# wolearyc/ramannoodle

Measured on AMD Instinct MI355X. Metric: structures/sec (GNN polarizability eval), higher is better.
Workload: dtype f32

## Files before the change

### ramannoodle_amd/csrc/api.hip

```cpp
#include <hip/hip_runtime.h>

#include <algorithm>
#include <chrono>
#include <cmath>
#include <cstdarg>
#include <cstdio>
#include <cstdlib>
#include <cstring>
#include <functional>
#include <memory>
#include <mutex>
#include <string>
#include <thread>
#include <vector>

#include "../../include/rn_potgnn.h"
#include "graph_plan.hpp"
#include "kernels.hpp"
#include "weight_layout.hpp"

using namespace rn;

namespace {

// ... 8 lines not shown
  do {                                                 \
    hipError_t _e = (expr);                            \
    if (_e != hipSuccess) throw HipError{_e, #expr};   \
  } while (0)

struct DeviceBuf {
  void *p = nullptr;
  size_t bytes = 0;
  ~DeviceBuf() { release(); }
  void release() {
    if (p) (void)hipFree(p);
    p = nullptr;
    bytes = 0;
  }
  void ensure(size_t n) {
    if (n <= bytes) return;
    release();
    HIP_TRY(hipMalloc(&p, n));
    bytes = n;
  }
  template <typename T>
  T *as() const { return reinterpret_cast<T *>(p); }
};

enum KernelId {
  K_GEOM = 0, K_NODE_INIT, K_PROJ_NODE, K_PROJ_EDGE_C1, K_NODE_AGG, K_PROJ_EDGE_C3, K_PROJ_C2,
  K_EDGE_AGG, K_READOUT_MLP, K_READOUT_REDUCE, K_C2_PAIRS, K_COUNT
};
const char *kKernelNames[K_COUNT] = {
    "geom_rbf", "node_init", "proj_node", "proj_edge_c1", "node_agg", "proj_edge_c3",
    "proj_c2", "edge_agg", "readout_mlp", "readout_reduce", "c2_pairs"};

template <typename T>
struct Lane {
  hipStream_t stream = nullptr;
  hipEvent_t done = nullptr;
  DeviceBuf unit4, node[2], edge[2], npc1, np3, bufA, bufB;
  DeviceBuf fbA, fbB;
};

template <typename T>
struct Precision {
  bool ready = false;
  DeviceBuf weights;
  DeviceBuf lattice;
  std::vector<PassW<T>> pass;
  ReadoutW<T> ro{};
  const T *offsets = nullptr, *node_table = nullptr, *ones = nullptr;
  Lane<T> lanes[2];
  std::vector<DeviceBuf> snap_node, snap_edge;
  std::vector<DeviceBuf> tape_node, tape_edge, tape_agg;
  DeviceBuf bw[18];
  hipStream_t side = nullptr;
  hipEvent_t ev_side[3] = {nullptr, nullptr, nullptr};
  DeviceBuf tn_arena;
  DeviceBuf tape_z1, bn_stats, grad, seeds, mv, type_sums;
  DeviceBuf in_dcart, in_lat, in_grads;
  DeviceBuf eye_seeds;
  int eye_frames = 0;
  bool tape_on = false;
};

struct TimedLaunch {
  int kid;
  hipEvent_t a, b;
};

}

struct rn_potgnn {
  mutable std::recursive_mutex lock;
  rn_potgnn_config cfg{};
  Dims d{};
  int chunk = 1;
  size_t f64_budget = 0;
  bool keep_stages = false;
  bool snap_pairs = false;
  bool last_pair_rows = false;
  bool debug_sync = false;
  GraphPlan plan;
  bool split_projections = true;
  bool want_pair_rows = true;
  bool want_c2_pairs = true;
  DeviceBuf step_seg, step_stage;
  float *step_host = nullptr;
  bool tape_ps = true;
  bool mfma_f16 = true;
  bool mfma_f16_requested = true;
  bool mfma_range_fallback = false;
  Graph g{};
  DeviceBuf g_ints;
  DeviceBuf ps_fail;
  double lattice[9], mean[9], stdv[9];
  DeviceBuf d_mean_std;
  std::vector<float> packed;
  PackedLayout lay;
  Precision<float> f32;
  Precision<double> f64;
  DeviceBuf io_pos, io_alpha, io_vec6, io_lat, io_types;
  struct Slot {
    DeviceBuf pos, alpha;
    hipEvent_t copied = nullptr, done = nullptr;
    bool busy = false;
  } slots[2];
  hipStream_t copy_stream = nullptr, exec_stream = nullptr;
  int next_slot = 0;
  struct HostStage {
    float *pin[2] = {nullptr, nullptr};
    size_t elems = 0;
    hipEvent_t copied[2] = {nullptr, nullptr};
    hipEvent_t done = nullptr;
    DeviceBuf pos;
    DeviceBuf lat;
    hipEvent_t caller = nullptr;
    char *out_pin = nullptr;
    size_t out_bytes = 0;
  } hstage;
  int last_chunk_structs = 0;
  int train_S = 0;
  int train_prec = 4;
  bool train_lat = false, train_types = false;
  bool tape_fused = true;
  bool device_training = false;
  bool grads_on_device = false;
  bool host_stale = false;
  DeviceBuf adam_m, adam_v, trainable_mask, derived_ops;
  int num_derived_ops = 0, derived_first_stage = 0;
  double bn_count = 0;
  rn_potgnn_reduce_fn reducer = nullptr;
  void *reducer_ctx = nullptr;
  bool last_was_f64 = false;
  bool last_in_order = false;
  int profiling = 0;
  std::vector<TimedLaunch> timed;
  double k_ms[K_COUNT] = {0};
  int64_t k_launches[K_COUNT] = {0};
  std::string error;
  hipEvent_t ev_start = nullptr;
  hipEvent_t ev_g[2] = {nullptr, nullptr};
  bool interleave = true;
  std::vector<int32_t> grp_labels;
  int grp_G = 0;
  DeviceBuf grp_csr, grp_jac, grp_disp, grp_out;
  DeviceBuf mode_vectors;
  DeviceBuf grp_jl, grp_lat, cells_lat;
};

namespace {

void set_error(rn_potgnn *h, const char *fmt, ...) {
  char buf[512];
  va_list ap;
  va_start(ap, fmt);
  vsnprintf(buf, sizeof(buf), fmt, ap);
  va_end(ap);
  if (h) {
    std::lock_guard<std::recursive_mutex> hold(h->lock);
    h->error = buf;
  } else {
    g_create_error = buf;
  }
}

bool lean_workspace(const rn_potgnn *h);
size_t per_structure_elems(const rn_potgnn *h, bool lean);
template <typename T>
// ... 266 lines not shown
    }
    cur = 0;
    snapshot(0);
  }

  void run_stages() {
    begin();
    for (int p = 0; p < h->cfg.num_message_passes; ++p) {
      stage_project(p);
      stage_aggregate(p);
    }
  }

  void project(const T *X, int64_t R, int K, const T *WT, int NOUT, T *Y, const T *bias, int amode, const T *nd) {
    if constexpr (sizeof(T) == 4) {
      if (h->mfma_f16 && h->split_projections &&
          launch_rowgemm_split(X, K, K, R, WT, NOUT, Y, false, bias, amode, nd, h->g, st()))
        return;
    }
    launch_rowgemm<T>(X, R, K, WT, NOUT, Y, nullptr, bias, false, amode, nd, h->g, st());
  }

  void stage_project(int p) {
    const PassW<T> &w = prec<T>(h).pass[p];
    const Graph &g = h->g;
    const Dims d = h->d;
    const int nxt = cur ^ 1;
    target_tape(p + 1, nxt);
    if constexpr (sizeof(T) == 4) {
      if (narrow()) {
        Timer t(h, st(), K_NODE_AGG);
        launch_node_narrow(edge[cur], node[cur], node[nxt], S, g, d, w, st());
        return;
      }
    }
    {
      Timer t(h, st(), K_PROJ_NODE);
      if (node_centred()) project(node[cur], MN, d.FnP, w.c1_WnT_c, 2 * d.FnP, npc1, w.c1_bias_c, 0, nullptr);
      else project(node[cur], MN, d.FnP, w.c1_WnT, 2 * d.FnP, npc1, w.c1_bias, 0, nullptr);
    }
    bool node_fused = false;
    if constexpr (sizeof(T) == 4) {
      if (fused() && h->plan.use_node_fused) {
        Timer t(h, st(), K_NODE_AGG);
        if (node_centred() && g.na_num > 0) launch_node_atom(edge[cur], node[cur], npc1, node[nxt], S, g, d, w, st(), pair_rows());
        else launch_node_fused(edge[cur], node[cur], npc1, node[nxt], S, g, d, w, h->mfma_f16, node_centred(), st());
        node_fused = true;
      }
    }
    if (!node_fused) {
      {
        Timer t(h, st(), K_PROJ_EDGE_C1);
        project(edge[cur], ME, d.FeP, w.c1_WeT, 2 * d.FnP, bufA, nullptr, 0, nullptr);
      }
      {
        Timer t(h, st(), K_NODE_AGG);
        launch_node_agg<T>(npc1, bufA, node[cur], node[nxt], S, g, d, w, st());
      }
    }
    {
      Timer t(h, st(), K_PROJ_NODE);
      if (role_split(w)) project(node[nxt], MN, d.FnP, w.c3_WnT_c, 6 * d.FeP, np3, w.c3_nshift_c, 0, nullptr);
      else project(node[nxt], MN, d.FnP, w.c3_WnT, 6 * d.FeP, np3, w.c3_nshift, 0, nullptr);
    }
    if (!fused()) {
      {
        Timer t(h, st(), K_PROJ_EDGE_C3);
        project(edge[cur], ME, d.FeP, w.c3_WeT, 4 * d.FeP, bufB, nullptr, 0, nullptr);
      }
      {
        Timer t(h, st(), K_PROJ_C2);
        project(nullptr, ME, d.FnP, w.c2_WT, 2 * d.FeP, bufA, w.c2_bias, 1, node[nxt]);
      }
    }
  }

  void stage_aggregate(int p) {
    const PassW<T> &w = prec<T>(h).pass[p];
    const int nxt = cur ^ 1;
    const float *c2_rows = nullptr;
    if constexpr (sizeof(T) == 4) {
      if (c2_pairs(w)) {
        Timer t(h, st(), K_C2_PAIRS);
        launch_c2_pairs(node[nxt], bufA, S, h->g, h->d, w, st());
        c2_rows = bufA;
      }
    }
    {
      Timer t(h, st(), K_EDGE_AGG);
      if constexpr (sizeof(T) == 4) {
        if (narrow()) launch_edge_narrow(edge[cur], edge[nxt], node[nxt], S, h->g, h->d, w, st());
        else if (role_split(w)) launch_edge_ps(edge[cur], edge[nxt], node[nxt], np3, tape_agg(p), S, h->g, h->d, w, h->ps_fail.as<int>(), st(), pair_rows(), h->mfma_f16, c2_rows);
        else if (fused()) edge_unfused_in_blocks(p);
        else HIP_TRY(launch_edge_agg<T>(bufB, np3, bufA, edge[cur], edge[nxt], S, h->g, h->d, w, tape_agg(p), st()));
      } else {
        HIP_TRY(launch_edge_agg<T>(bufB, np3, bufA, edge[cur], edge[nxt], S, h->g, h->d, w, tape_agg(p), st()));
      }
    }
    cur = nxt;
    snapshot(p + 1);
  }

  void edge_unfused_in_blocks(int p) {
    const PassW<T> &w = prec<T>(h).pass[p];
    const Graph &g = h->g;
    const Dims d = h->d;
    const int nxt = cur ^ 1;
    const size_t per_frame = (size_t)g.E * (size_t)(6 * d.FeP) * sizeof(T);
    int block = (int)std::max<size_t>(1, std::min<size_t>((size_t)S, ((size_t)1 << 30) / std::max<size_t>(per_frame, 1)));
    if (const char *e = getenv("RN_POTGNN_UNFUSED_BLOCK_FRAMES")) block = std::max(1, std::min(block, atoi(e)));
    ln->fbA.ensure((size_t)block * g.E * 2 * d.FeP * sizeof(T));
    ln->fbB.ensure((size_t)block * g.E * 4 * d.FeP * sizeof(T));
    T *fa = ln->fbA.template as<T>(), *fb = ln->fbB.template as<T>();
    T *agg = tape_agg(p);
    for (int s0 = 0; s0 < S; s0 += block) {
      const int sb = std::min(block, S - s0);
      const int64_t rows = (int64_t)sb * g.E;
      const T *e_in = edge[cur] + (size_t)s0 * g.E * d.FeP, *nd = node[nxt] + (size_t)s0 * g.N * d.FnP;
      project(e_in, rows, d.FeP, w.c3_WeT, 4 * d.FeP, fb, nullptr, 0, nullptr);
      project(nullptr, rows, d.FnP, w.c2_WT, 2 * d.FeP, fa, w.c2_bias, 1, nd);
      HIP_TRY(launch_edge_agg<T>(fb, np3 + (size_t)s0 * g.N * 6 * d.FeP, fa, e_in, edge[nxt] + (size_t)s0 * g.E * d.FeP, sb, g, d, w,
                                 agg ? agg + (size_t)s0 * g.E * d.FeP : nullptr, st()));
    }
  }

  void finish() {
    Precision<T> &P = prec<T>(h);
    const Graph &g = h->g;
    const Dims d = h->d;
    if constexpr (sizeof(T) == 4) {
      if (narrow()) {
        Timer t(h, st(), K_READOUT_MLP);
        const double *ms = h->d_mean_std.as<double>();
        launch_readout_narrow(edge[cur], unit4, S, g, d, P.ro, ms, ms + 9, io.vec6, io.alpha, io.alpha_raw,
                              h->keep_stages ? bufA : nullptr, st());
        HIP_TRY(hipGetLastError());
        return;
      }
    }
    int pol_stride = 32;
    {
      Timer t(h, st(), K_READOUT_MLP);
      const int HP = std::max(d.FeP, 32);
      bool done = false;
      if constexpr (sizeof(T) == 4) {
        if (fused() && h->plan.use_readout_fused) {
          pol_stride = h->keep_stages ? 32 : 16;
          launch_readout_fused(edge[cur], ME, P.ro, bufA, h->mfma_f16, st(), pair_rows(), pol_stride);
          done = true;
        }
      }
      if (!done) {
        launch_rowgemm<T>(edge[cur], ME, d.FeP, P.ro.W0T, HP, bufA, P.ro.scale0, P.ro.shift0, true, 0,
                          nullptr, g, st());
        launch_rowgemm<T>(bufA, ME, HP, P.ro.W3T, HP, bufB, P.ones, P.ro.b3, true, 0, nullptr, g, st());
        launch_rowgemm<T>(bufB, ME, HP, P.ro.W5T, 32, bufA, nullptr, P.ro.b5, false, 0, nullptr, g,
                          st());
      }
    }
    {
      Timer t(h, st(), K_READOUT_REDUCE);
      const double *ms = h->d_mean_std.as<double>();
      launch_readout_reduce<T>(bufA, unit4, S, g, ms, ms + 9, io.vec6, io.alpha, io.alpha_raw, st(), pol_stride);
    }
    HIP_TRY(hipGetLastError());
  }
  bool fused() const { return sizeof(T) == 4 && h->plan.use_fused && (!prec<T>(h).tape_on || h->tape_fused); }
// ... 946 lines not shown
               o_nt = push(plan.nt.begin), o_bt = push(plan.bt.begin), o_pt = push(plan.pt.begin), o_ipos = push(plan.in_pos),
               o_pe = push(plan.pair_of_edge), o_pa = push(plan.pair_a), o_pb = push(plan.pair_b);
  buf.ensure(ints.size() * sizeof(int));
  HIP_TRY(hipMemcpy(buf.p, ints.data(), ints.size() * sizeof(int), hipMemcpyHostToDevice));
  const int *base = buf.as<int>();
  Graph g = plan.scalars();
  g.edge_a = base + o_a;
  g.edge_b = base + o_b;
  g.out_ptr = base + o_op;
  g.in_ptr = base + o_ip;
  g.in_edge = base + o_ie;
  g.in_pos = base + o_ipos;
  g.atom_type = base + o_at;
  g.rev_edge = base + o_rv;
  g.pair_of_edge = base + o_pe;
  g.pair_a = base + o_pa;
  g.pair_b = base + o_pb;
  g.tile_begin = base + o_tb;
  g.trip_off = base + o_to;
  g.nt_begin = base + o_nt;
  g.pt_begin = base + o_pt;
  g.bt_begin = base + o_bt;
  return g;
}

static void size_chunk(rn_potgnn *h) {
  int chunk = h->cfg.max_chunk_structures;
  if (const char *e = getenv("RN_POTGNN_CHUNK")) chunk = atoi(e);
  if (chunk <= 0) {
    const size_t per = per_structure_elems(h, lean_workspace(h)) * sizeof(float);
    size_t budget = (h->plan.use_fused || h->plan.use_narrow) ? ((size_t)8192 << 20) : ((size_t)1536 << 20);
    size_t free_b = 0, total_b = 0;
    if (hipMemGetInfo(&free_b, &total_b) == hipSuccess && free_b > 0)
      budget = std::min(budget, std::max<size_t>(free_b / 8 / (size_t)h->plan.num_lanes, (size_t)64 << 20));
    chunk = (int)std::max<size_t>(1, budget / std::max<size_t>(per, 1));
    chunk = std::min(chunk, 4096);
    h->f64_budget = (size_t)24 << 30;
    if (free_b > 0) h->f64_budget = std::min(h->f64_budget, std::max<size_t>(free_b / 8 / (size_t)h->plan.num_lanes, (size_t)64 << 20));
  }
  h->chunk = chunk;
}

int rn_potgnn_create(const rn_potgnn_config *cfg, const int32_t *edge_a, const int32_t *edge_b,
                     const int32_t *atom_types, const double *lattice, const float *weights,
                     size_t num_weights, const double *mean, const double *stddev,
                     rn_potgnn **out) {
  if (!out) return RN_ERR_INVALID_ARGUMENT;
  *out = nullptr;
  std::string invalid;
  int rc = validate_create_args(cfg, edge_a, edge_b, atom_types, !lattice || !weights || !mean || !stddev, &num_weights, invalid);
  if (rc != RN_OK) {
    set_error(nullptr, "%s", invalid.c_str());
    return rc;
  }

  int ndev = 0;
  if (hipGetDeviceCount(&ndev) != hipSuccess || ndev <= 0 || cfg->device < 0 ||
      cfg->device >= ndev) {
    set_error(nullptr, "no usable HIP device (count=%d, requested=%d)", ndev, cfg->device);
    return RN_ERR_NO_DEVICE;
  }
  int cus = 256;
  {
    hipDeviceProp_t prop;
    if (hipGetDeviceProperties(&prop, cfg->device) == hipSuccess && prop.multiProcessorCount > 0) cus = prop.multiProcessorCount;
  }

  std::unique_ptr<rn_potgnn> h(new rn_potgnn());
  h->cfg = *cfg;
  std::memcpy(h->lattice, lattice, sizeof(h->lattice));
  std::memcpy(h->mean, mean, sizeof(h->mean));
  std::memcpy(h->stdv, stddev, sizeof(h->stdv));
  h->snap_pairs = getenv("RN_POTGNN_KEEP_STAGES") && atoi(getenv("RN_POTGNN_KEEP_STAGES")) == 2;
  h->keep_stages = getenv("RN_POTGNN_KEEP_STAGES") && atoi(getenv("RN_POTGNN_KEEP_STAGES")) != 0 && !h->snap_pairs;
  h->debug_sync = getenv("RN_POTGNN_DEBUG_SYNC") && atoi(getenv("RN_POTGNN_DEBUG_SYNC")) != 0;
  if (const char *e = getenv("RN_POTGNN_INTERLEAVE")) h->interleave = atoi(e) != 0;
  if (const char *e = getenv("RN_POTGNN_MFMA")) h->mfma_f16_requested = !(e[0] == 'f' && e[1] == '3');
  h->mfma_f16 = h->mfma_f16_requested;
  if (const char *e = getenv("RN_POTGNN_TAPE_FUSED")) h->tape_fused = atoi(e) != 0;
  if (const char *e = getenv("RN_POTGNN_TAPE_PS")) h->tape_ps = atoi(e) != 0;
  h->split_projections = getenv("RN_POTGNN_SPLIT_PROJ") ? atoi(getenv("RN_POTGNN_SPLIT_PROJ")) != 0 : true;
  h->want_pair_rows = !(getenv("RN_POTGNN_PAIR_ROWS") && atoi(getenv("RN_POTGNN_PAIR_ROWS")) == 0);
  h->want_c2_pairs = !(getenv("RN_POTGNN_C2_PAIRS") && atoi(getenv("RN_POTGNN_C2_PAIRS")) == 0);

  const PlanKnobs knobs = read_plan_knobs();
  h->d = plan_dims(*cfg, knobs);
  h->plan = plan_graph(*cfg, h->d, edge_a, edge_b, atom_types, cus, knobs);

  rn_potgnn *hp = h.get();
  rc = guarded(nullptr, [&]() {
    HIP_TRY(hipSetDevice(cfg->device));
    HIP_TRY(hipEventCreateWithFlags(&hp->ev_start, hipEventDisableTiming));
    HIP_TRY(hipEventCreateWithFlags(&hp->ev_g[0], hipEventDisableTiming));
    HIP_TRY(hipEventCreateWithFlags(&hp->ev_g[1], hipEventDisableTiming));
    hp->g = upload(hp->plan, hp->g_ints);
    double ms[18];
    std::memcpy(ms, hp->mean, sizeof(hp->mean));
    std::memcpy(ms + 9, hp->stdv, sizeof(hp->stdv));
    hp->d_mean_std.ensure(sizeof(ms));
    HIP_TRY(hipMemcpy(hp->d_mean_std.p, ms, sizeof(ms), hipMemcpyHostToDevice));
    hp->lay = layout_weights(hp->cfg, hp->d);
    pack_weights(hp->lay, weights, hp->packed);
    refresh_mfma_mode(hp);
    hp->ps_fail.ensure(2048);
    HIP_TRY(hipMemset(hp->ps_fail.p, 0, 2048));
    size_chunk(hp);
    ensure_precision<float>(hp);
  });
  if (rc != RN_OK) return rc;
  *out = h.release();
  return RN_OK;
}

int rn_potgnn_debug_plan(const rn_potgnn_config *cfg, const int32_t *edge_a, const int32_t *edge_b,
                         const int32_t *atom_types, int32_t num_cus, int32_t *out, size_t capacity, size_t *count) {
  if (!count || num_cus <= 0) return RN_ERR_INVALID_ARGUMENT;
  *count = 0;
  std::string invalid;
  const int rc = validate_create_args(cfg, edge_a, edge_b, atom_types, false, nullptr, invalid);
  if (rc != RN_OK) {
    set_error(nullptr, "%s", invalid.c_str());
    return rc;
  }
  try {
    const PlanKnobs knobs = read_plan_knobs();
    const std::vector<int32_t> flat = plan_graph(*cfg, plan_dims(*cfg, knobs), edge_a, edge_b, atom_types, num_cus, knobs).flat();
    *count = flat.size();
    if (!out || capacity < flat.size()) {
      set_error(nullptr, "out holds %zu values, the plan has %zu", out ? capacity : (size_t)0, flat.size());
      return RN_ERR_INVALID_ARGUMENT;
    }
    std::memcpy(out, flat.data(), flat.size() * sizeof(int32_t));
    return RN_OK;
  } catch (const std::bad_alloc &) {
    set_error(nullptr, "host allocation failed");
    return RN_ERR_OUT_OF_MEMORY;
  }
}

int rn_potgnn_debug_plan_pairs(const rn_potgnn_config *cfg, const int32_t *edge_a, const int32_t *edge_b,
                               const int32_t *atom_types, int32_t num_cus, int32_t *out, size_t capacity, size_t *count) {
  if (!count || num_cus <= 0) return RN_ERR_INVALID_ARGUMENT;
  *count = 0;
  std::string invalid;
  const int rc = validate_create_args(cfg, edge_a, edge_b, atom_types, false, nullptr, invalid);
  if (rc != RN_OK) {
    set_error(nullptr, "%s", invalid.c_str());
    return rc;
  }
  try {
    const PlanKnobs knobs = read_plan_knobs();
    const std::vector<int32_t> flat = plan_graph(*cfg, plan_dims(*cfg, knobs), edge_a, edge_b, atom_types, num_cus, knobs).flat_pairs();
    *count = flat.size();
    if (!out || capacity < flat.size()) {
      set_error(nullptr, "out holds %zu values, the pair table has %zu", out ? capacity : (size_t)0, flat.size());
      return RN_ERR_INVALID_ARGUMENT;
    }
    std::memcpy(out, flat.data(), flat.size() * sizeof(int32_t));
    return RN_OK;
  } catch (const std::bad_alloc &) {
    set_error(nullptr, "host allocation failed");
    return RN_ERR_OUT_OF_MEMORY;
  }
}

int rn_potgnn_debug_plan_lds(const rn_potgnn_config *cfg, const int32_t *edge_a, const int32_t *edge_b,
// ... 1083 lines not shown
```

### ramannoodle_amd/csrc/graph_plan.hip

```cpp
#include "graph_plan.hpp"

#include <algorithm>
#include <cstdarg>
#include <cstdio>
#include <cstdlib>

namespace rn {

namespace {

std::string format(const char *fmt, ...) {
  char buf[512];
  va_list ap;
  va_start(ap, fmt);
  vsnprintf(buf, sizeof(buf), fmt, ap);
  va_end(ap);
  return buf;
}

const char *knob(const char *name) { return getenv(name); }
bool knob_flag(const char *name, bool otherwise) { return knob(name) ? atoi(knob(name)) != 0 : otherwise; }

void widen_for_fused(Dims &d, int widen) {
  if (widen == 0) return;
// ... 297 lines not shown
}

size_t max_out_degree(Dims d) {
  size_t deg = 0;
  while (edge_agg_f64_lds_bytes(d, (int)deg + 1, (int)deg + 1, 1) <= kCuLdsBytes) ++deg;
  return deg;
}

int validate_config(const rn_potgnn_config *cfg_in, bool others_null, const size_t *num_weights, std::string &error) {
  if (!cfg_in || others_null) {
    error = "null argument";
    return RN_ERR_INVALID_ARGUMENT;
  }
  const rn_potgnn_config &cfg = *cfg_in;
  const int N = cfg.num_atoms, E = cfg.num_edges;
  if (N <= 0 || E < 0 || cfg.num_atom_types <= 0 || cfg.size_node_embedding <= 0 ||
      cfg.size_edge_embedding <= 0 || cfg.num_message_passes <= 0) {
    error = "invalid configuration (non-positive size)";
    return RN_ERR_INVALID_ARGUMENT;
  }
  if (E == 0) {
    error = "reference graph has no edges: the per-structure mean over edges "
            "(_gnn.py:662-664) is undefined";
    return RN_ERR_INVALID_ARGUMENT;
  }
  if (cfg.size_node_embedding > 128 || cfg.size_edge_embedding > 128) {
    error = format("embedding sizes above 128 are not supported (Fn=%d, Fe=%d)", cfg.size_node_embedding,
                   cfg.size_edge_embedding);
    return RN_ERR_UNSUPPORTED;
  }
  if (num_weights && *num_weights != rn_potgnn_weight_count(&cfg)) {
    error = format("weights has %zu floats, expected %zu", *num_weights, rn_potgnn_weight_count(&cfg));
    return RN_ERR_INVALID_ARGUMENT;
  }
  return RN_OK;
}

int validate_create_args(const rn_potgnn_config *cfg_in, const int32_t *edge_a, const int32_t *edge_b, const int32_t *atom_types,
                         bool others_null, const size_t *num_weights, std::string &error) {
  const bool graph_null = !atom_types || (cfg_in && cfg_in->num_edges > 0 && (!edge_a || !edge_b));
  if (const int rc = validate_config(cfg_in, others_null || graph_null, num_weights, error); rc != RN_OK) return rc;
  const rn_potgnn_config &cfg = *cfg_in;
  const int N = cfg.num_atoms, E = cfg.num_edges;
  for (int e = 0; e < E; ++e) {
    if (edge_a[e] < 0 || edge_a[e] >= N || edge_b[e] < 0 || edge_b[e] >= N || edge_a[e] == edge_b[e]) {
      error = format("edge %d = (%d,%d) is out of range or a self loop", e, edge_a[e], edge_b[e]);
      return RN_ERR_INVALID_ARGUMENT;
    }
    if (e > 0 && (edge_a[e] < edge_a[e - 1] || (edge_a[e] == edge_a[e - 1] && edge_b[e] <= edge_b[e - 1]))) {
      error = format("edges must be strictly sorted by (a, b); violated at edge %d", e);
      return RN_ERR_INVALID_ARGUMENT;
    }
  }
  for (int n = 0; n < N; ++n)
    if (atom_types[n] < 0 || atom_types[n] >= cfg.num_atom_types) {
      error = format("atom %d has type %d outside [0,%d)", n, atom_types[n], cfg.num_atom_types);
      return RN_ERR_INVALID_ARGUMENT;
    }
  const Dims d = plan_dims(cfg, read_plan_knobs());
  const size_t cap = max_out_degree(d);
  std::vector<int> deg(N, 0), deg_in(N, 0);
  for (int e = 0; e < E; ++e) deg[edge_a[e]]++, deg_in[edge_b[e]]++;
  for (int n = 0; n < N; ++n)
    if ((size_t)deg[n] > cap) {
      error = format("atom %d has %d outgoing edges; more than %zu per atom is unsupported "
                     "for size_edge_embedding=%d", n, deg[n], cap, cfg.size_edge_embedding);
      return RN_ERR_UNSUPPORTED;
    }
  const int max_out = *std::max_element(deg.begin(), deg.end()), max_in = *std::max_element(deg_in.begin(), deg_in.end());
  const size_t need = edge_agg_f64_lds_bytes(d, max_out, max_in, 1);
  if (need > kCuLdsBytes) {
    error = format("an atom with %d outgoing edges beside one with %d incoming edges needs %zu bytes of LDS per tile in "
                   "float64 (%zu available) for size_edge_embedding=%d", max_out, max_in, need, kCuLdsBytes, cfg.size_edge_embedding);
    return RN_ERR_UNSUPPORTED;
  }
  return RN_OK;
}

GraphPlan plan_graph(const rn_potgnn_config &cfg, Dims d, const int32_t *edge_a, const int32_t *edge_b,
                     const int32_t *atom_types, int num_cus, const PlanKnobs &k) {
  GraphPlan g;
  g.N = cfg.num_atoms;
  g.E = cfg.num_edges;
  g.d = d;
  g.edge_a.assign(edge_a, edge_a + g.E);
  g.edge_b.assign(edge_b, edge_b + g.E);
  g.atom_type.assign(atom_types, atom_types + g.N);
  build_index_arrays(g);

  const bool fused_mode = k.want_fused && d.FnP == 64 && d.FeP == 64;
  const bool narrow_mode = k.want_narrow && narrow_supported(d);
  g.tile = edge_tiles(g, k, fused_mode, narrow_mode);
  if (edge_agg_f64_lds_bytes(d, g.tile.max_out_rows, g.tile.max_in_rows, g.tile.max_nodes) > kCuLdsBytes) g.tile = one_atom_tiles(g);
  if (k.bwd_tiles) g.bt = reverse_tiles(g);
  if (narrow_mode) g.nt = node_tiles_narrow(g, k);
  g.nt_narrow = g.nt.num() > 0;
  if (!g.nt_narrow) g.nt = node_tiles_wide(g, k);
  if (fused_mode && k.want_ps) g.pt = ps_tiles(g, k, num_cus, &g.pt_back, &g.pt_gram);
  choose_node_atom(g, k);

  const Graph s = g.scalars();
  g.use_fused = k.want_fused && edge_fused_supported(s, d);
  g.use_ps = g.use_fused && g.pt.num() > 0;
  g.use_narrow = narrow_mode && edge_narrow_lds_bytes(d.Fn, d.Fe, g.tile.max_out_rows, g.tile.max_in_rows) <= (size_t)64 * 1024;
  g.use_node_fused = g.use_fused && k.want_node_fused && node_fused_lds_bytes(s) <= 64 * 1024;
  g.use_readout_fused = g.use_fused && k.want_readout_fused;
  g.num_lanes = k.lanes > 0 ? k.lanes : ((g.use_fused || g.use_narrow) ? 1 : 2);
  return g;
}

Graph GraphPlan::scalars() const {
  Graph s{};
  s.N = N, s.E = E, s.T = T;
  s.NP = (int)pair_a.size();
  s.num_tiles = tile.num(), s.max_tile_out_rows = tile.max_out_rows, s.max_tile_in_rows = tile.max_in_rows, s.max_tile_nodes = tile.max_nodes;
  s.nt_num = nt.num(), s.nt_max_in_rows = nt.max_in_rows, s.nt_max_nodes = nt.max_nodes, s.nt_narrow = nt_narrow ? 1 : 0;
  s.na_num = na_num, s.na_max_deg = na_max_deg;
  s.pt_num = pt.num(), s.pt_max_out_rows = pt.max_out_rows, s.pt_max_in_rows = pt.max_in_rows, s.pt_back = pt_back, s.pt_gram = pt_gram;
  s.bt_num = bt.num(), s.bt_max_out_rows = bt.max_out_rows, s.bt_max_in_rows = bt.max_in_rows, s.bt_max_nodes = bt.max_nodes;
  return s;
}

std::vector<int64_t> GraphPlan::lds_requests() const {
  const Graph s = scalars();
  const bool node_fused = use_fused && use_node_fused;
  std::vector<int64_t> o;
  auto add = [&o](size_t f32, size_t f64) { o.insert(o.end(), {(int64_t)f32, (int64_t)f64}); };
  add(edge_agg_lds_bytes(s, d, sizeof(float)), edge_agg_lds_bytes(s, d, sizeof(double)));
  add(edge_bwd_lds_bytes(s, d.FeP, sizeof(float)), edge_bwd_lds_bytes(s, d.FeP, sizeof(double)));
  add(use_narrow ? edge_narrow_lds_bytes(d.Fn, d.Fe, tile.max_out_rows, tile.max_in_rows) : 0, 0);
  add(use_narrow && nt_narrow ? node_tiled_lds_bytes(d.Fn, d.Fe, nt.max_in_rows, nt.max_nodes) : 0, 0);
  add(use_ps ? edge_ps_lds_bytes(pt.max_out_rows, pt.max_in_rows, pt_gram != 0) : 0, 0);
  add(node_fused && na_num > 0 ? node_atom_lds_bytes(na_max_deg) : 0, 0);
  add(node_fused ? node_fused_lds_bytes(s) : 0, 0);
  return o;
}

std::vector<int32_t> GraphPlan::flat() const {
  std::vector<int32_t> o = {d.FnP, d.FeP};
  const Partition reserved;
  for (const Partition *p : {&tile, &nt, &reserved, &bt, &pt}) {
    o.push_back((int32_t)p->begin.size());
    o.insert(o.end(), p->begin.begin(), p->begin.end());
    o.insert(o.end(), {p->max_out_rows, p->max_in_rows, p->max_nodes});
  }
  o.insert(o.end(), {nt_narrow ? 1 : 0, na_num, na_max_deg, pt_back, pt_gram, (int32_t)T});
  o.insert(o.end(), {use_fused, 0 , 0 , use_ps, use_narrow, use_node_fused, use_readout_fused, num_lanes});
  for (const std::vector<int> *v : {&out_ptr, &in_ptr, &in_edge, &in_pos, &rev_edge, &trip_off}) o.insert(o.end(), v->begin(), v->end());
  return o;
}

std::vector<int32_t> GraphPlan::flat_pairs() const {
  std::vector<int32_t> o = {(int32_t)pair_a.size()};
  for (const std::vector<int> *v : {&pair_of_edge, &pair_a, &pair_b}) o.insert(o.end(), v->begin(), v->end());
  return o;
}

}
```

### ramannoodle_amd/csrc/graph_plan.hpp

```cpp
#pragma once

#include <string>
#include <vector>

#include "../../include/rn_potgnn.h"
#include "kernels.hpp"

namespace rn {

struct PlanKnobs {
  int widen = 2;
  bool vpl8 = false;
  bool want_fused = true;
  bool want_narrow = true;
  bool tile_kb_set = false;
  int tile_kb = 64;
  int narrow_tile_rows = 0;
  bool bwd_tiles = true;
  bool node_tile_rows_set = false;
  int node_tile_rows = 0;
  int node_tile_kb = 12;
  bool want_ps = true;
  int ps_tile_rows = 0;
  int ps_back = 5;
  bool want_gram = false;
  int node_atom = -1;
  bool want_node_fused = true;
  bool want_readout_fused = true;
  int lanes = 0;
};
PlanKnobs read_plan_knobs();

int pad_pow2(int f);
Dims plan_dims(const rn_potgnn_config &cfg, const PlanKnobs &knobs);
size_t max_out_degree(Dims d);

int validate_config(const rn_potgnn_config *cfg, bool others_null, const size_t *num_weights, std::string &error);
int validate_create_args(const rn_potgnn_config *cfg, const int32_t *edge_a, const int32_t *edge_b, const int32_t *atom_types,
                         bool others_null, const size_t *num_weights, std::string &error);

struct Partition {
  std::vector<int> begin;
  int max_out_rows = 0, max_in_rows = 0, max_nodes = 0;
  int num() const { return begin.empty() ? 0 : (int)begin.size() - 1; }
};

struct GraphPlan {
  int N = 0, E = 0;
  Dims d{};
  std::vector<int> edge_a, edge_b, atom_type;
  std::vector<int> out_ptr, in_ptr;
  std::vector<int> in_edge, in_pos;
  std::vector<int> rev_edge;
  std::vector<int> trip_off;
  std::vector<int> pair_of_edge;
  std::vector<int> pair_a, pair_b;
  int64_t T = 0;
  Partition tile, nt, bt, pt;
  bool nt_narrow = false;
  int na_num = 0, na_max_deg = 0;
  int pt_back = 2, pt_gram = 0;
  bool use_fused = false;
  bool use_ps = false;
  bool use_narrow = false;
  bool use_node_fused = false;
  bool use_readout_fused = false;
  int num_lanes = 2;

  Graph scalars() const;
  std::vector<int64_t> lds_requests() const;
  std::vector<int32_t> flat() const;
  std::vector<int32_t> flat_pairs() const;
};

GraphPlan plan_graph(const rn_potgnn_config &cfg, Dims d, const int32_t *edge_a, const int32_t *edge_b,
                     const int32_t *atom_types, int num_cus, const PlanKnobs &knobs);

}
```

### ramannoodle_amd/csrc/kernels.hpp

```cpp
#pragma once
#include <hip/hip_runtime.h>
#include <algorithm>
#include <cstddef>
#include <cstdint>
#include <vector>

namespace rn {

struct Graph {
  int N, E;
  const int *edge_a;
  const int *edge_b;
  const int *out_ptr;
  const int *in_ptr;
  const int *in_edge;
  const int *in_pos;
  const int *atom_type;
  const int *rev_edge;
  int NP;
  const int *pair_of_edge;
  const int *pair_a, *pair_b;
  int num_tiles;
  const int *tile_begin;
  int max_tile_out_rows;
// ... 194 lines not shown
template <typename T>
void launch_bn_bwd_sums(const T *d, const T *z, int64_t R, int W, int F, const double *stats, double count,
                        double *sums, hipStream_t st);
template <typename T>
void launch_bn_bwd_apply(T *d, const T *z, int64_t R, int W, int F, const double *stats, double count,
                         const double *sums, const double *own_sums, const T *gamma, T *dgamma, T *dbeta,
                         hipStream_t st);
template <typename T>
void launch_node_embed_bwd(const T *dnode0, int S, const Graph &g, Dims d, int K, const T *emb,
                           const T *W2, const T *b2, const T *W4, T *demb, T *dW2, T *db2, T *dW4,
                           T *db4, T *type_sums_scratch,
                           const int *types , hipStream_t st);
template <typename T>
void launch_geom_bwd(const T *dedge0, const T *dunit, const T *unit4, const T *lat, const T *offs,
                     T coef, int C, int B, const Graph &g, Dims d, double *dpos, hipStream_t st);
template <typename T>
void launch_geom_input_bwd(const T *dedge0, const T *dunit, const T *unit4, const double *pos, const T *lat,
                           int lat_stride, const T *offs, T coef, int C, int B, const Graph &g, Dims d, double *dcart,
                           double *dpos, double *dlat, hipStream_t st);
template <typename T>
void launch_cast_from_f64(const double *src, T *dst, int64_t n, hipStream_t st);
constexpr int kMaxGroups = 16;

void launch_group_increments(const double *jac, int64_t jac_stride, const double *pos, const double *disp,
                             double disp_scale, int64_t steps, int N, const int *perm, const int *gptr, int G,
                             const double *sigma, double *out, hipStream_t st, int out_groups = 0);
void launch_cell_increments(const double *jl, const double *lat, int64_t steps, int channel, int out_groups,
                            const double *sigma, double *out, hipStream_t st);
constexpr int kMaxModes = 64 * 65535;
void launch_mode_increments(const double *jac, const double *pos, int64_t steps, int N, const double *disp,
                            const double *proj, int M, const double *sigma, int out_channels, double *out,
                            hipStream_t st);
void launch_mode_rest(const double *jac, const double *pos, int64_t steps, int N, int M, const double *sigma,
                      int out_channels, double *out, hipStream_t st);

struct InterpModel {
  const double *F, *FT, *ref, *alpha_ref, *xs, *coef, *scale;
  const int *poff;
  int64_t K3;
  int J, order, Pmax;
};
void launch_interp_alpha(const double *pos, int64_t S, const InterpModel &m, double *alpha, hipStream_t st);
void launch_interp_jacobian(const double *pos, int64_t S, const InterpModel &m, double *g, double *jac, hipStream_t st);
inline bool group_csr(const int32_t *labels, int N, int G, std::vector<int32_t> &csr) {
  std::vector<int32_t> ptr(G + 1, 0);
  for (int i = 0; i < N; ++i) {
    if (labels[i] < 0 || labels[i] >= G) return false;
    ++ptr[labels[i] + 1];
  }
  for (int g = 0; g < G; ++g) {
    if (ptr[g + 1] == 0) return false;
    ptr[g + 1] += ptr[g];
  }
  csr.assign((size_t)N + G + 1, 0);
  std::vector<int32_t> fill(ptr.begin(), ptr.end() - 1);
  for (int i = 0; i < N; ++i) csr[fill[labels[i]]++] = i;
  std::copy(ptr.begin(), ptr.end(), csr.begin() + N);
  return true;
}

constexpr size_t kFusedLdsBudget = 80 * 1024;
size_t edge_fused_lds_bytes(const Graph &g);
size_t edge_fused_lds_bytes(int tile_out_rows, int tile_in_rows, int tile_nodes);
bool edge_fused_supported(const Graph &g, Dims d);
size_t node_fused_lds_bytes(const Graph &g);
size_t node_fused_lds_bytes(int tile_in_rows, int tile_nodes);
void launch_readout_fused(const float *edge, int64_t M, const ReadoutW<float> &w, float *pol, bool f16,
                          hipStream_t st, bool pair_rows = false, int pol_stride = 32 );
size_t node_atom_lds_bytes(int max_deg);
void launch_node_atom(const float *edge, const float *node_in, const float *npc1, float *node_out, int S, const Graph &g,
                      Dims d, const PassW<float> &w, hipStream_t st, bool pair_rows = false);
void launch_node_fused(const float *edge, const float *node_in, const float *npc1, float *node_out, int S,
                       const Graph &g, Dims d, const PassW<float> &w, bool f16, bool centred, hipStream_t st);
size_t edge_ps_lds_bytes(int tile_out_rows, int tile_in_rows, bool gram);
int edge_ps_ring_tiles(bool gram);
int edge_ps_gram_window();
bool edge_ps_tile_ok(const int *rb, const int *re, int D, int back, int ring, int *window);
void launch_edge_ps(const float *edge_in, float *edge_out, const float *node, const float *np3, float *agg_out, int S,
                    const Graph &g, Dims d, const PassW<float> &w, int *fail, hipStream_t st, bool pair_rows = false,
                    bool f16 = true ,
                    const float *c2_rows = nullptr );
bool edge_ps_takes_c2_rows(const Graph &g, bool pair_rows, bool f16);

void launch_c2_pairs(const float *node, float *out, int S, const Graph &g, Dims d, const PassW<float> &w, hipStream_t st);

struct DerivedOp {
  int kind;
  int K, N;
  float scale;
  size_t src, dst;
  int Fe = 0, FeP = 0;
};
void launch_adam(float *w, const float *g, float *m, float *v, const unsigned char *trainable, size_t n,
                 double lr, double beta1, double beta2, double eps, double weight_decay, int64_t step,
                 hipStream_t st, const int *poisoned = nullptr );
void launch_refresh_derived(float *w, const DerivedOp *ops, int num_ops, hipStream_t st);
void launch_gather_segments(const float *w, const long long *seg, int nseg, float *staging, hipStream_t st);
void launch_bn_running(float *running_mean, float *running_var, const float *batch_mean, const float *batch_var,
                       int F, double momentum, double unbias, hipStream_t st);

bool narrow_supported(Dims d);
size_t edge_narrow_lds_bytes(int fn, int fe, int tile_out_rows, int tile_in_rows);
size_t node_tiled_lds_bytes(int fn, int fe, int tile_in_rows, int tile_nodes);
void launch_node_narrow(const float *edge, const float *node_in, float *node_out, int S, const Graph &g, Dims d,
                        const PassW<float> &w, hipStream_t st);
void launch_edge_narrow(const float *edge_in, float *edge_out, const float *node, int S, const Graph &g, Dims d,
                        const PassW<float> &w, hipStream_t st);
void launch_readout_narrow(const float *edge, const float *unit4, int S, const Graph &g, Dims d,
                           const ReadoutW<float> &w, const double *mean9, const double *std9, float *vec6,
                           double *alpha, double *alpha_raw, float *pol , hipStream_t st);

}
```

### ramannoodle_amd/csrc/kernels_c2_pairs.hip

```cpp
#include "fused_common.hpp"

namespace rn {

struct C2PairArgs {
  const float *node;
  float *out;
  int64_t M;
  int N, NP;
  const int *pair_a, *pair_b;
  Dims d;
  PassW<float> w;
};

namespace {
constexpr int C2P_THREADS = 256;
}

__global__ __launch_bounds__(C2P_THREADS, 2) void c2_pairs_kernel(C2PairArgs a) {
  __shared__ __attribute__((aligned(16))) float s_bias[2 * FP], s_g1[2 * FP], s_b1[2 * FP], s_g2[FP], s_b2[FP];
  const int tid = threadIdx.x, lane = tid & 63, wave = tid >> 6;
  const int l15 = lane & 15, quad = lane >> 4;
  const float sc2 = a.w.mfma_scale_c[4];
  for (int c = tid; c < 2 * FP; c += C2P_THREADS) {
    s_bias[c] = a.w.c2_bias_c[c] * sc2;
    s_g1[c] = a.w.c2_norm_1.g[c];
    s_b1[c] = a.w.c2_norm_1.b[c];
    if (c < FP) {
      s_g2[c] = a.w.c2_norm_2.g[c];
      s_b2[c] = a.w.c2_norm_2.b[c];
    }
  }
  WaveB<true> bW[4];
#pragma unroll
  for (int p = 0; p < 4; ++p) bW[p].load(a.w.c2_WT_c, 2 * FP, 32 * p, l15, quad, sc2);
  __syncthreads();

  const float inv2n = 1.0f / (float)(2 * a.d.Fe), invn = 1.0f / (float)a.d.Fe;
  const float eps_c2 = 1e-5f * sc2 * sc2;
  const int64_t ntiles = (a.M + 15) / 16, stride = (int64_t)gridDim.x * (C2P_THREADS / 64);

  f32x4 xb[4], xa[4];
  auto fetch = [&](int64_t tile) {
    int64_t row = tile * 16 + l15;
    if (row >= a.M) row = a.M - 1;
    const int64_t s = row / a.NP;
    const int p = (int)(row - s * a.NP);
    const float *nb = a.node + (s * a.N + a.pair_b[p]) * FP + 16 * quad, *na = a.node + (s * a.N + a.pair_a[p]) * FP + 16 * quad;
#pragma unroll
    for (int j = 0; j < 4; ++j) {
      xb[j] = *reinterpret_cast<const f32x4 *>(nb + 4 * j);
      xa[j] = *reinterpret_cast<const f32x4 *>(na + 4 * j);
    }
  };
  int64_t tile = (int64_t)blockIdx.x * (C2P_THREADS / 64) + wave;
  if (tile < ntiles) fetch(tile);
  for (; tile < ntiles; tile += stride) {
    float af[KS];
#pragma unroll
    for (int j = 0; j < 4; ++j) {
      const f32x4 pr = xb[j] * xa[j];
#pragma unroll
      for (int i = 0; i < 4; ++i) af[4 * j + i] = pr[i];
    }
    f16x8 ah[2], al[2];
    split_f16x8(af, ah[0], al[0]);
    split_f16x8(af + 8, ah[1], al[1]);
    if (tile + stride < ntiles) fetch(tile + stride);

    const int lq = launder(lane >> 4);
    f32x4 acc[4][2];
#pragma unroll
    for (int p = 0; p < 4; ++p) {
#pragma unroll
      for (int t = 0; t < 2; ++t) acc[p][t] = *reinterpret_cast<const f32x4 *>(s_bias + 32 * p + 16 * t + 4 * lq);
      bW[p].product_split(ah, al, acc[p]);
    }
    float q = 0.f;
#pragma unroll
    for (int p = 0; p < 4; ++p)
#pragma unroll
      for (int t = 0; t < 2; ++t)
#pragma unroll
        for (int i = 0; i < 4; ++i) q = fmaf(acc[p][t][i], acc[p][t][i], q);
    q = sum_xor32(sum_xor16(q));
    const float rstd2 = fast_rsq(q * inv2n + eps_c2);
    float gv[2][2][4], sum = 0.f;
#pragma unroll
    for (int p = 0; p < 2; ++p)
#pragma unroll
      for (int t = 0; t < 2; ++t) {
        const int c = 32 * p + 16 * t + 4 * lq;
        const Vec4<float> gf = load4<float>(s_g1 + c), bf = load4<float>(s_b1 + c);
        const Vec4<float> gc = load4<float>(s_g1 + FP + c), bc = load4<float>(s_b1 + FP + c);
#pragma unroll
        for (int i = 0; i < 4; ++i) {
          gv[p][t][i] = gate(acc[p][t][i] * rstd2 * gf.v[i] + bf.v[i], acc[p + 2][t][i] * rstd2 * gc.v[i] + bc.v[i]);
          sum += gv[p][t][i];
        }
      }
    const float mean = sum_xor32(sum_xor16(sum)) * invn;
    float qq = 0.f;
#pragma unroll
    for (int p = 0; p < 2; ++p)
#pragma unroll
      for (int t = 0; t < 2; ++t)
#pragma unroll
        for (int i = 0; i < 4; ++i) {
          const int c = 32 * p + 16 * t + 4 * lq + i;
          gv[p][t][i] = c < a.d.Fe ? gv[p][t][i] - mean : 0.f;
          qq = fmaf(gv[p][t][i], gv[p][t][i], qq);
        }
    const float rstd = fast_rsq(sum_xor32(sum_xor16(qq)) * invn + 1e-5f);
    const int64_t row = tile * 16 + l15;
    if (row < a.M) {
#pragma unroll
      for (int p = 0; p < 2; ++p)
#pragma unroll
        for (int t = 0; t < 2; ++t) {
          const int c = 32 * p + 16 * t + 4 * lq;
          const Vec4<float> g2 = load4<float>(s_g2 + c), b2 = load4<float>(s_b2 + c);
          f32x4 y;
#pragma unroll
          for (int i = 0; i < 4; ++i) y[i] = gv[p][t][i] * rstd * g2.v[i] + b2.v[i];
          *reinterpret_cast<f32x4 *>(a.out + row * FP + c) = y;
        }
    }
  }
}

void launch_c2_pairs(const float *node, float *out, int S, const Graph &g, Dims d, const PassW<float> &w, hipStream_t st) {
  const int64_t M = (int64_t)S * g.NP;
  if (M == 0) return;
  C2PairArgs a{node, out, M, g.N, g.NP, g.pair_a, g.pair_b, d, w};
  static int cus = 0;
  if (cus == 0) {
    int dev = 0;
    hipDeviceProp_t prop;
    if (hipGetDevice(&dev) == hipSuccess && hipGetDeviceProperties(&prop, dev) == hipSuccess) cus = prop.multiProcessorCount;
    if (cus <= 0) cus = 256;
  }
  const int64_t ntiles = (M + 15) / 16, per_wg = C2P_THREADS / 64;
  const int64_t grid = std::min<int64_t>((ntiles + per_wg - 1) / per_wg, (int64_t)2 * cus);
  c2_pairs_kernel<<<(unsigned)grid, C2P_THREADS, 0, st>>>(a);
}

}
```

Measured before the change: 64740.

## Stage c2 pair weights in LDS to raise occupancy and simplify indexing

The c2_pairs kernel now loads the split-f16 weight fragments cooperatively into shared memory, with each wave loading one 32-column group, instead of every wave holding all four groups in registers. This frees VGPRs so launch bounds can go from 2 to 4 blocks, and the grid cap rises to match. Row-to-pair index math is made incremental, replacing a per-tile 64-bit division. A PAD template drops the column mask when Fe equals FeP. The cost is extra LDS reads of the weights inside the MFMA loop and more shared memory per block.

```diff
diff --git a/ramannoodle_amd/csrc/api.hip b/ramannoodle_amd/csrc/api.hip
--- a/ramannoodle_amd/csrc/api.hip
+++ b/ramannoodle_amd/csrc/api.hip
@@ -114,6 +114,7 @@
   bool split_projections = true;
   bool want_pair_rows = true;
   bool want_c2_pairs = true;
+  int c2_pairs_grid = 0;
   DeviceBuf step_seg, step_stage;
   float *step_host = nullptr;
   bool tape_ps = true;
@@ -546,7 +547,7 @@
     if constexpr (sizeof(T) == 4) {
       if (c2_pairs(w)) {
         Timer t(h, st(), K_C2_PAIRS);
-        launch_c2_pairs(node[nxt], bufA, S, h->g, h->d, w, st());
+        launch_c2_pairs(node[nxt], bufA, S, h->g, h->d, w, h->plan.num_cus, h->c2_pairs_grid, st());
         c2_rows = bufA;
       }
     }
@@ -1659,6 +1660,7 @@
   h->split_projections = getenv("RN_POTGNN_SPLIT_PROJ") ? atoi(getenv("RN_POTGNN_SPLIT_PROJ")) != 0 : true;
   h->want_pair_rows = !(getenv("RN_POTGNN_PAIR_ROWS") && atoi(getenv("RN_POTGNN_PAIR_ROWS")) == 0);
   h->want_c2_pairs = !(getenv("RN_POTGNN_C2_PAIRS") && atoi(getenv("RN_POTGNN_C2_PAIRS")) == 0);
+  if (const char *e = getenv("RN_POTGNN_C2_PAIRS_GRID")) h->c2_pairs_grid = std::max(0, atoi(e));
 
   const PlanKnobs knobs = read_plan_knobs();
   h->d = plan_dims(*cfg, knobs);
diff --git a/ramannoodle_amd/csrc/graph_plan.hip b/ramannoodle_amd/csrc/graph_plan.hip
--- a/ramannoodle_amd/csrc/graph_plan.hip
+++ b/ramannoodle_amd/csrc/graph_plan.hip
@@ -403,6 +403,7 @@
   GraphPlan g;
   g.N = cfg.num_atoms;
   g.E = cfg.num_edges;
+  g.num_cus = num_cus;
   g.d = d;
   g.edge_a.assign(edge_a, edge_a + g.E);
   g.edge_b.assign(edge_b, edge_b + g.E);
diff --git a/ramannoodle_amd/csrc/graph_plan.hpp b/ramannoodle_amd/csrc/graph_plan.hpp
--- a/ramannoodle_amd/csrc/graph_plan.hpp
+++ b/ramannoodle_amd/csrc/graph_plan.hpp
@@ -47,6 +47,7 @@
 
 struct GraphPlan {
   int N = 0, E = 0;
+  int num_cus = 0;
   Dims d{};
   std::vector<int> edge_a, edge_b, atom_type;
   std::vector<int> out_ptr, in_ptr;
diff --git a/ramannoodle_amd/csrc/kernels.hpp b/ramannoodle_amd/csrc/kernels.hpp
--- a/ramannoodle_amd/csrc/kernels.hpp
+++ b/ramannoodle_amd/csrc/kernels.hpp
@@ -300,7 +300,8 @@
                     const float *c2_rows = nullptr );
 bool edge_ps_takes_c2_rows(const Graph &g, bool pair_rows, bool f16);
 
-void launch_c2_pairs(const float *node, float *out, int S, const Graph &g, Dims d, const PassW<float> &w, hipStream_t st);
+void launch_c2_pairs(const float *node, float *out, int S, const Graph &g, Dims d, const PassW<float> &w, int num_cus, int grid_cap,
+                     hipStream_t st);
 
 struct DerivedOp {
   int kind;
diff --git a/ramannoodle_amd/csrc/kernels_c2_pairs.hip b/ramannoodle_amd/csrc/kernels_c2_pairs.hip
--- a/ramannoodle_amd/csrc/kernels_c2_pairs.hip
+++ b/ramannoodle_amd/csrc/kernels_c2_pairs.hip
@@ -6,7 +6,7 @@
   const float *node;
   float *out;
   int64_t M;
-  int N, NP;
+  int S, N, NP;
   const int *pair_a, *pair_b;
   Dims d;
   PassW<float> w;
@@ -14,11 +14,17 @@
 
 namespace {
 constexpr int C2P_THREADS = 256;
+constexpr int C2P_WAVES = C2P_THREADS / 64;
+constexpr int C2P_WAVES_PER_SIMD = 4;
+static_assert(C2P_WAVES == 4,"one wave per 32-column group of the 128 pre-activation columns");
+__device__ __forceinline__ constexpr int c2p_frag(int p, int t, int s, int half) { return ((p * 2 + t) * 2 + s) * 2 + half; }
 }
 
-__global__ __launch_bounds__(C2P_THREADS, 2) void c2_pairs_kernel(C2PairArgs a) {
+template <bool PAD>
+__global__ __launch_bounds__(C2P_THREADS, C2P_WAVES_PER_SIMD) void c2_pairs_kernel(C2PairArgs a) {
   __shared__ __attribute__((aligned(16))) float s_bias[2 * FP], s_g1[2 * FP], s_b1[2 * FP], s_g2[FP], s_b2[FP];
-  const int tid = threadIdx.x, lane = tid & 63, wave = tid >> 6;
+  __shared__ __attribute__((aligned(16))) f16x8 s_w[32][64];
+  const int tid = threadIdx.x, lane = tid & 63, wave = __builtin_amdgcn_readfirstlane(tid >> 6);
   const int l15 = lane & 15, quad = lane >> 4;
   const float sc2 = a.w.mfma_scale_c[4];
   for (int c = tid; c < 2 * FP; c += C2P_THREADS) {
@@ -30,30 +36,54 @@
       s_b2[c] = a.w.c2_norm_2.b[c];
     }
   }
-  WaveB<true> bW[4];
+  {
+    WaveB<true> bW;
+    bW.load(a.w.c2_WT_c, 2 * FP, 32 * wave, l15, quad, sc2);
 #pragma unroll
-  for (int p = 0; p < 4; ++p) bW[p].load(a.w.c2_WT_c, 2 * FP, 32 * p, l15, quad, sc2);
+    for (int t = 0; t < 2; ++t)
+#pragma unroll
+      for (int s = 0; s < 2; ++s) {
+        s_w[c2p_frag(wave, t, s, 0)][lane] = bW.h[t][s];
+        s_w[c2p_frag(wave, t, s, 1)][lane] = bW.l[t][s];
+      }
+  }
   __syncthreads();
 
   const float inv2n = 1.0f / (float)(2 * a.d.Fe), invn = 1.0f / (float)a.d.Fe;
   const float eps_c2 = 1e-5f * sc2 * sc2;
-  const int64_t ntiles = (a.M + 15) / 16, stride = (int64_t)gridDim.x * (C2P_THREADS / 64);
+  const int64_t ntiles = (a.M + 15) / 16, stride = (int64_t)gridDim.x * C2P_WAVES;
+  const int64_t d_row = stride * 16;
+  const int d_s = (int)(d_row / a.NP), d_p = (int)(d_row - (int64_t)d_s * a.NP);
+  const int64_t d_sn = (int64_t)d_s * a.N, last_sn = (int64_t)(a.S - 1) * a.N;
 
   f32x4 xb[4], xa[4];
-  auto fetch = [&](int64_t tile) {
-    int64_t row = tile * 16 + l15;
-    if (row >= a.M) row = a.M - 1;
+  int64_t tile = (int64_t)blockIdx.x * C2P_WAVES + wave;
+  int64_t row = tile * 16 + l15, sn;
+  int pair;
+  {
     const int64_t s = row / a.NP;
-    const int p = (int)(row - s * a.NP);
-    const float *nb = a.node + (s * a.N + a.pair_b[p]) * FP + 16 * quad, *na = a.node + (s * a.N + a.pair_a[p]) * FP + 16 * quad;
+    pair = (int)(row - s * a.NP);
+    sn = s * a.N;
+  }
+  auto fetch = [&]() {
+    const bool in = row < a.M;
+    const int64_t fsn = in ? sn : last_sn;
+    const int fp = in ? pair : a.NP - 1;
+    const float *nb = a.node + (fsn + a.pair_b[fp]) * FP + 16 * quad, *na = a.node + (fsn + a.pair_a[fp]) * FP + 16 * quad;
 #pragma unroll
     for (int j = 0; j < 4; ++j) {
       xb[j] = *reinterpret_cast<const f32x4 *>(nb + 4 * j);
       xa[j] = *reinterpret_cast<const f32x4 *>(na + 4 * j);
     }
+    row += d_row;
+    sn += d_sn;
+    pair += d_p;
+    if (pair >= a.NP) {
+      pair -= a.NP;
+      sn += a.N;
+    }
   };
-  int64_t tile = (int64_t)blockIdx.x * (C2P_THREADS / 64) + wave;
-  if (tile < ntiles) fetch(tile);
+  if (tile < ntiles) fetch();
   for (; tile < ntiles; tile += stride) {
     float af[KS];
 #pragma unroll
@@ -65,15 +95,21 @@
     f16x8 ah[2], al[2];
     split_f16x8(af, ah[0], al[0]);
     split_f16x8(af + 8, ah[1], al[1]);
-    if (tile + stride < ntiles) fetch(tile + stride);
+    const int64_t orow = row - d_row;
+    fetch();
 
     const int lq = launder(lane >> 4);
+    const f16x8 *wl = &s_w[0][0] + launder(lane);
     f32x4 acc[4][2];
 #pragma unroll
     for (int p = 0; p < 4; ++p) {
 #pragma unroll
       for (int t = 0; t < 2; ++t) acc[p][t] = *reinterpret_cast<const f32x4 *>(s_bias + 32 * p + 16 * t + 4 * lq);
-      bW[p].product_split(ah, al, acc[p]);
+#pragma unroll
+      for (int s = 0; s < 2; ++s)
+#pragma unroll
+        for (int t = 0; t < 2; ++t)
+          acc[p][t] = mfma_split3_t<(RN_MFMA_K32 != 0)>(wl[64 * c2p_frag(p, t, s, 0)], wl[64 * c2p_frag(p, t, s, 1)], ah[s], al[s], acc[p][t]);
     }
     float q = 0.f;
 #pragma unroll
@@ -107,12 +143,11 @@
 #pragma unroll
         for (int i = 0; i < 4; ++i) {
           const int c = 32 * p + 16 * t + 4 * lq + i;
-          gv[p][t][i] = c < a.d.Fe ? gv[p][t][i] - mean : 0.f;
+          gv[p][t][i] = !PAD || c < a.d.Fe ? gv[p][t][i] - mean : 0.f;
           qq = fmaf(gv[p][t][i], gv[p][t][i], qq);
         }
     const float rstd = fast_rsq(sum_xor32(sum_xor16(qq)) * invn + 1e-5f);
-    const int64_t row = tile * 16 + l15;
-    if (row < a.M) {
+    if (orow < a.M) {
 #pragma unroll
       for (int p = 0; p < 2; ++p)
 #pragma unroll
@@ -122,26 +157,22 @@
           f32x4 y;
 #pragma unroll
           for (int i = 0; i < 4; ++i) y[i] = gv[p][t][i] * rstd * g2.v[i] + b2.v[i];
-          *reinterpret_cast<f32x4 *>(a.out + row * FP + c) = y;
+          *reinterpret_cast<f32x4 *>(a.out + orow * FP + c) = y;
         }
     }
   }
 }
 
-void launch_c2_pairs(const float *node, float *out, int S, const Graph &g, Dims d, const PassW<float> &w, hipStream_t st) {
+void launch_c2_pairs(const float *node, float *out, int S, const Graph &g, Dims d, const PassW<float> &w, int num_cus, int grid_cap,
+                     hipStream_t st) {
   const int64_t M = (int64_t)S * g.NP;
   if (M == 0) return;
-  C2PairArgs a{node, out, M, g.N, g.NP, g.pair_a, g.pair_b, d, w};
-  static int cus = 0;
-  if (cus == 0) {
-    int dev = 0;
-    hipDeviceProp_t prop;
-    if (hipGetDevice(&dev) == hipSuccess && hipGetDeviceProperties(&prop, dev) == hipSuccess) cus = prop.multiProcessorCount;
-    if (cus <= 0) cus = 256;
-  }
-  const int64_t ntiles = (M + 15) / 16, per_wg = C2P_THREADS / 64;
-  const int64_t grid = std::min<int64_t>((ntiles + per_wg - 1) / per_wg, (int64_t)2 * cus);
-  c2_pairs_kernel<<<(unsigned)grid, C2P_THREADS, 0, st>>>(a);
+  C2PairArgs a{node, out, M, S, g.N, g.NP, g.pair_a, g.pair_b, d, w};
+  const int64_t ntiles = (M + 15) / 16;
+  int64_t grid = std::min<int64_t>((ntiles + C2P_WAVES - 1) / C2P_WAVES, (int64_t)C2P_WAVES_PER_SIMD * (num_cus > 0 ? num_cus : 256));
+  if (grid_cap > 0) grid = std::min<int64_t>(grid, grid_cap);
+  auto kern = d.Fe != d.FeP ? &c2_pairs_kernel<true> : &c2_pairs_kernel<false>;
+  kern<<<(unsigned)grid, C2P_THREADS, 0, st>>>(a);
 }
 
 }
```

After: 64860, median of 6. About the same (+0.2%).
